# twesterhout/annealing-sign-problem

Hardware: AMD Instinct MI355X
Metric: SA spin-flips/sec, kagome_36-sized clusters (higher is better)
Workload: dtype f64

## Files before the change

annealing_sign_problem_amd/_lib.py:

```python
from __future__ import annotations

import atexit
import ctypes
import os
import sys
import weakref
from typing import Optional

import numpy as np

from . import build as _build

c_void_p = ctypes.c_void_p
c_u64 = ctypes.c_uint64
c_u32 = ctypes.c_uint32
c_i32 = ctypes.c_int32
c_int = ctypes.c_int
c_float = ctypes.c_float
c_double = ctypes.c_double


class AspError(RuntimeError):

    def __init__(self, code: int, message: str):
# ... 187 lines not shown
                                       ctypes.c_double, c_u64, c_void_p, ctypes.POINTER(c_u64),
                                       c_u64, c_void_p, c_void_p, c_void_p, ctypes.POINTER(c_u64)]),
    "asp_sparsify_last_ms": (c_float, []),
    "asp_sa_plan_create": (c_void_p, [c_u64, c_void_p, c_void_p, c_void_p, c_void_p]),
    "asp_sa_plan_destroy": (None, [c_void_p]),
    "asp_sa_plan_info": (c_int, [c_void_p, ctypes.POINTER(SaInfo)]),
    "asp_sa_layout_host": (c_int, [c_u64, c_void_p, c_void_p, c_void_p, c_void_p,
                                   ctypes.POINTER(SaInfo), c_void_p, c_void_p]),
    "asp_sa_layout_build_count": (c_u64, []),
    "asp_sa_plan_reweight": (c_int, [c_void_p, c_u64, c_void_p, c_void_p, c_void_p, c_void_p]),
    "asp_sa_plan_reweight_last_ms": (c_float, [c_void_p]),
    "asp_sa_plan_clone": (c_int, [c_void_p, ctypes.POINTER(c_void_p)]),
    "asp_sa_batch_slots_host": (c_int, [c_u32, c_void_p, c_void_p, ctypes.POINTER(c_u32), c_void_p, c_u64]),
    "asp_sa_shuffled_order_host": (c_int, [c_u64, c_void_p, c_void_p, c_void_p, c_void_p, c_u64, c_u32,
                                           c_void_p, c_void_p, ctypes.POINTER(c_u32)]),
    "asp_sa_set_launch": (c_int, [c_void_p, c_int, c_int]),
    "asp_sa_set_packed": (c_int, [c_void_p, c_int]),
    "asp_sa_set_wide": (c_int, [c_void_p, c_int]),
    "asp_sa_set_team": (c_int, [c_void_p, c_int]),
    "asp_sa_last_layout": (c_int, [c_void_p]),
    "asp_sa_set_lds_limit": (c_int, [c_void_p, c_u64]),
    "asp_sa_last_spin_layout": (c_int, [c_void_p]),
    "asp_sa_set_field_cache": (c_int, [c_void_p, c_int]),
    "asp_sa_set_post": (c_int, [c_void_p, c_int]),
    "asp_sa_anneal": (c_int, [c_void_p, c_u64, c_void_p, c_u32, c_u32, c_u32, c_void_p, c_void_p,
                              c_void_p]),
    "asp_sa_anneal_trace": (c_int, [c_void_p, c_u64, c_void_p, c_u32, c_u32, c_u32, c_void_p,
                                    c_void_p, c_void_p, c_void_p]),
    "asp_sa_anneal_shuffled": (c_int, [c_void_p, c_u64, c_void_p, c_u32, c_u32, c_u32, c_void_p, c_void_p,
                                       c_void_p]),
    "asp_sa_anneal_shuffled_trace": (c_int, [c_void_p, c_u64, c_void_p, c_u32, c_u32, c_u32, c_void_p,
                                             c_void_p, c_void_p, c_void_p]),
    "asp_sa_set_shuffled_launch": (c_int, [c_void_p, c_int, c_int]),
    "asp_sa_set_shuffled_teams": (c_int, [c_void_p, c_int]),
    "asp_sa_last_shuffled": (c_int, [c_void_p, ctypes.POINTER(c_u32), ctypes.POINTER(c_float)]),
    "asp_sa_team_watchdog_trips": (c_int, [c_void_p, ctypes.POINTER(c_u32), ctypes.POINTER(c_u64)]),
    "asp_sa_last_shuffled_blocks": (c_int, [c_void_p, ctypes.POINTER(c_u32), ctypes.POINTER(c_u32)]),
    "asp_sa_last_shuffled_fill": (c_int, [c_void_p, ctypes.POINTER(ctypes.c_double), ctypes.POINTER(ctypes.c_double)]),
    "asp_sa_chains_create": (c_int, [c_void_p, c_u64, c_u32, c_u32, c_void_p, c_u64, ctypes.POINTER(c_void_p)]),
    "asp_sa_chains_destroy": (None, [c_void_p]),
    "asp_sa_chains_advance": (c_int, [c_void_p, c_void_p, c_u32, c_u32, c_void_p]),
    "asp_sa_chains_result": (c_int, [c_void_p, c_void_p, c_void_p]),
    "asp_sa_chains_export": (c_int, [c_void_p, ctypes.POINTER(SaChainsSnapshot)]),
    "asp_sa_chains_import": (c_int, [c_void_p, ctypes.POINTER(SaChainsSnapshot)]),
    "asp_sa_chains_advance_batch": (c_int, [ctypes.POINTER(SaChainsItem), c_u32]),
    "asp_sa_chains_batch_last_ms": (c_float, []),
    "asp_sa_chains_gather": (c_int, [c_void_p, c_void_p]),
    "asp_sa_chains_resample": (c_int, [c_void_p, c_double, c_u32, c_void_p, c_void_p, c_void_p, c_void_p]),
# ... 170 lines not shown
```

annealing_sign_problem_amd/annealer.py:

```python
from __future__ import annotations

import ctypes
import os
from typing import Optional, Tuple

import numpy as np
import scipy.sparse

from . import _lib

__all__ = [
    "Hamiltonian",
    "PatternMismatch",
    "anneal",
    "anneal_batch",
    "anneal_traces",
    "anneal_until",
    "Chains",
    "resample_chains",
    "population_anneal",
    "population_anneal_batch",
    "parallel_tempering",
    "parallel_tempering_batch",
    "parallel_tempering_cluster",
# ... 218 lines not shown
def _resolve_seed(seed) -> int:
    if seed is None:
        return int.from_bytes(os.urandom(8), "little")
    return int(seed) & (2**64 - 1)


def anneal_raw(hamiltonian: Hamiltonian, seed: int, betas: np.ndarray, repetitions: int,
               replica_offset: int = 0, x0=None, shuffled: bool = False):
    lib = _lib.load()
    plan = hamiltonian.plan()
    words = (hamiltonian.size + 63) // 64
    betas = np.ascontiguousarray(betas, dtype=np.float64)
    xs = np.zeros((repetitions, max(words, 1)), dtype=np.uint64)
    es = np.zeros(repetitions, dtype=np.float64)
    if x0 is not None:
        x0 = np.ascontiguousarray(x0, dtype=np.uint64).reshape(-1)
        if x0.shape[0] != words:
            raise ValueError("'x0' must have {} words".format(words))
    entry = lib.asp_sa_anneal_shuffled if shuffled else lib.asp_sa_anneal
    _lib.check(entry(plan, ctypes.c_uint64(seed), _lib.ptr(betas),
                     ctypes.c_uint32(betas.shape[0]), ctypes.c_uint32(repetitions),
                     ctypes.c_uint32(replica_offset), _lib.ptr(x0), _lib.ptr(xs), _lib.ptr(es)))
    return xs[:, :words], es


def anneal_raw_into(hamiltonian: Hamiltonian, seed: int, betas: np.ndarray, repetitions: int,
                    replica_offset: int, x0, out_x_ptr: int, out_e_ptr: int,
                    shuffled: bool = False) -> None:
    lib = _lib.load()
    betas = np.ascontiguousarray(betas, dtype=np.float64)
    if x0 is not None:
        x0 = np.ascontiguousarray(x0, dtype=np.uint64).reshape(-1)
        if x0.shape[0] != (hamiltonian.size + 63) // 64:
            raise ValueError("'x0' must have {} words".format((hamiltonian.size + 63) // 64))
    entry = lib.asp_sa_anneal_shuffled if shuffled else lib.asp_sa_anneal
    _lib.check(entry(hamiltonian.plan(), ctypes.c_uint64(seed), _lib.ptr(betas),
                     ctypes.c_uint32(betas.shape[0]), ctypes.c_uint32(repetitions),
                     ctypes.c_uint32(replica_offset), _lib.ptr(x0),
                     ctypes.c_void_p(out_x_ptr), ctypes.c_void_p(out_e_ptr)))


def anneal(hamiltonian: Hamiltonian, x0=None, seed=None, number_sweeps: int = 5120,
           beta0: Optional[float] = None, beta1: Optional[float] = None, repetitions: int = 1,
           only_best: bool = True, distributed: bool = True, sweep_order: Optional[str] = None):
    if not isinstance(hamiltonian, Hamiltonian):
        raise TypeError("'hamiltonian' must be a Hamiltonian")
# ... 762 lines not shown
```

annealing_sign_problem_amd/csrc/sa_internal.hpp:

```cpp
#pragma once

#include <hip/hip_runtime.h>

#include <algorithm>
#include <atomic>
#include <cstdint>
#include <memory>
#include <mutex>
#include <utility>
#include <vector>

#include "asp_common.hpp"
#include "sa_plan.hpp"

namespace asp {

struct SaPattern {
  uint64_t nnz = 0;
  std::vector<int64_t> indptr;
  std::vector<int32_t> indices;
  std::mutex build;
  bool built = false;
  static constexpr uint32_t kNone = 0xFFFFFFFFu;
  std::vector<uint32_t> src_ij, src_ji;
// ... 30 lines not shown
  size_t spin_lds() const { return spin_lds_limit ? std::min(spin_lds_limit, max_lds) : max_lds; }
  asp::DeviceBuffer<uint32_t> color_block_start, block_width, ell_col, spin_of_pos, pos_of_spin;
  asp::DeviceBuffer<uint32_t> ell_col4;
  int last_layout = 0;
  int last_spin_layout = 0;
  asp::DeviceBuffer<uint64_t> ell_off;
  asp::DeviceBuffer<double> ell_val, field_pos;
  asp::DeviceBuffer<double> w_betas, w_partial, w_e;
  asp::DeviceBuffer<uint64_t> w_best, w_x0, w_x0_perm, w_x;
  asp::DeviceBuffer<long long> w_tracked;
  asp::DeviceBuffer<unsigned long long> w_accepted;
  asp::DeviceBuffer<double> w_field_cache;
  asp::DeviceBuffer<uint64_t> w_spins;
  asp::DeviceBuffer<long long> w_trace;
  asp::DeviceBuffer<uint64_t> w_cur_perm;
  asp::DeviceBuffer<long long> w_e_cur;
  void *team_area = nullptr;
  size_t team_area_bytes = 0;
  ~asp_sa_plan() {
    if (team_area) (void)hipFree(team_area);
  }
  int team_mode = -1;
  bool use_field_cache = true;
  bool use_post = true;
  uint32_t team_abort_host = 0;
  uint32_t team_watchdog_trips = 0;
  asp::DeviceBuffer<uint32_t> rq_ptr;
  asp::DeviceBuffer<uint32_t> rq_col;
  asp::DeviceBuffer<double> rq_val;
  asp::DeviceBuffer<double> field_dev;
  uint32_t rq_quads = 0, rq_max_quads = 0;
  int shuffled_m = 0, shuffled_waves = 0;
  int shuffled_teams = 0;
  int last_shuffled_levels = 0;
  uint32_t last_shuffled_log_s = 6, last_shuffled_wgs = 0;
  uint32_t last_shuffled_blocks = 0, last_shuffled_quads = 0;
  float last_order_ms = 0.0f;
  asp::DeviceBuffer<uint32_t> cluster_row_ptr, cluster_col;
  asp::DeviceBuffer<double> cluster_val, cluster_field;
  asp::DeviceBuffer<uint32_t> cluster_scratch;
  int greedy_tree = 0;
};


struct asp_sa_chains {
  asp_sa_plan *plan = nullptr;
// ... 99 lines not shown
```

annealing_sign_problem_amd/csrc/sa_reweight.hip:

```cpp
#include <hip/hip_runtime.h>

#include <algorithm>
#include <cmath>
#include <cstring>
#include <limits>
#include <vector>

#include "asp_common.hpp"
#include "sa_internal.hpp"

namespace {

using asp::SaPattern;

constexpr uint32_t kNone = SaPattern::kNone;
constexpr int kThreads = 256;

__global__ __launch_bounds__(kThreads) void k_rw_merge(const double *__restrict__ data,
                                                       const uint32_t *__restrict__ src_ij,
                                                       const uint32_t *__restrict__ src_ji, uint64_t entries,
                                                       double *__restrict__ staged, uint32_t *zeros) {
  const uint64_t stride = static_cast<uint64_t>(gridDim.x) * kThreads;
  for (uint64_t e = static_cast<uint64_t>(blockIdx.x) * kThreads + threadIdx.x; e < entries; e += stride) {
    const uint32_t a = src_ij[e], b = src_ji[e];
// ... 284 lines not shown
  ASP_HIP_TRY(hipEventElapsedTime(&p->rw_last_ms, p->ev[0], p->ev[3]));
  return ASP_OK;
}

float asp_sa_plan_reweight_last_ms(asp_sa_plan const *p) { return p ? p->rw_last_ms : 0.0f; }

int asp_sa_plan_clone(asp_sa_plan const *p, asp_sa_plan **out) {
  asp_clear_error();
  if (!p) return asp::set_error(ASP_ERR_INVALID, "null plan");
  if (!out) return asp::set_error(ASP_ERR_INVALID, "null output pointer");
  *out = nullptr;
  ASP_TRY(asp::bind_device());
  asp_sa_plan *c = new (std::nothrow) asp_sa_plan();
  if (!c) return asp::set_error(ASP_ERR_ALLOC, "out of host memory");
  c->host = p->host;
  c->pattern = p->pattern;
  c->force_m = p->force_m;
  c->force_threads = p->force_threads;
  c->force_packed = p->force_packed;
  c->spin_lds_limit = p->spin_lds_limit;
  c->allow_wide = p->allow_wide;
  c->team_mode = p->team_mode;
  c->use_field_cache = p->use_field_cache;
  c->use_post = p->use_post;
  c->shuffled_m = p->shuffled_m;
  c->shuffled_waves = p->shuffled_waves;
  c->shuffled_teams = p->shuffled_teams;
  c->greedy_tree = p->greedy_tree;
  const int rc = asp::sa_plan_device_setup(c);
  if (rc != ASP_OK) {
    asp_sa_plan_destroy(c);
    return rc;
  }
  *out = c;
  return ASP_OK;
}

}
```

annealing_sign_problem_amd/csrc/sa_sweep.hip:

```cpp
#include <algorithm>
#include <atomic>
#include <chrono>
#include <cmath>
#include <cstdlib>
#include <initializer_list>
#include <memory>
#include <mutex>
#include <numeric>
#include <type_traits>
#include <vector>

#include "asp_common.hpp"
#include "greedy.hpp"
#include "sa_device.hpp"
#include "sa_internal.hpp"
#include "sa_plan.hpp"

namespace {

using asp::DeviceBuffer;
using asp::kDummySpin;
using asp::upload_vector;
using namespace asp::dev;

// ... 311 lines not shown
  __device__ __forceinline__ double of(int, double beta) const { return beta; }
};
template <int M>
struct LadderBetas<M, true> {
  static constexpr bool kHeld = M <= 2;
  double own[kHeld ? M : 1];
  const double *mine;
  __device__ __forceinline__ LadderBetas(const ResumeLadder &res, uint32_t group)
      : mine(res.chain_betas + static_cast<uint64_t>(group) * M) {
    if constexpr (kHeld) {
#pragma unroll
      for (int m = 0; m < M; ++m) own[m] = mine[m];
    }
  }
  __device__ __forceinline__ double of(int m, double) const {
    if constexpr (kHeld) {
      return own[m];
    } else {
      return mine[m];
    }
  }
};

template <int M, bool DESCENT, int LAYOUT, typename Args, typename Stop = NoEarlyStop,
          typename Res = NoResume, bool ALIGNED = false>
__device__ __forceinline__ void sa_sweep_body(const Args &a, const uint32_t group,
                                              const Stop stop = Stop{}, const Res res = Res{}) {
  static_assert(DESCENT || !Stop::kEnabled, "only a descent can stop early");
  static_assert(!ALIGNED || (!DESCENT && M == 4), "an aligned group is one whole Philox call");
  static_assert(!DESCENT || !Res::kEnabled, "a descent is never resumed");
  constexpr bool GLOBAL = LAYOUT == kGlobal;
  constexpr bool PACKED = LAYOUT == kBits || GLOBAL;
  constexpr bool WIDE = LAYOUT == kWide;
  constexpr bool NIBBLES = LAYOUT == kNibbles;
  constexpr bool kLeanBook = M <= 4 && !(Res::kLadder && WIDE);
  static_assert(!PACKED || M == 1, "the bit-packed layouts hold one replica");
  static_assert(!NIBBLES || (M <= 4 && !DESCENT), "the nibble layout holds up to four replicas");
  static_assert(!WIDE || (M <= 4 && !DESCENT), "the wide layout holds up to four replicas");
  extern __shared__ __align__(16) uint8_t lds[];
  uint8_t *spins = GLOBAL ? reinterpret_cast<uint8_t *>(a.spin_words +
                                                       static_cast<uint64_t>(group) * a.num_blocks)
                          : lds;
  const uint32_t P = GLOBAL ? 0u : a.num_blocks * (PACKED ? 8u : (WIDE ? 256u : (NIBBLES ? 32u : 64u)));
  long long *delta = reinterpret_cast<long long *>(lds + P);
  long long *book = delta + 8;
  uint32_t *improved_flag = reinterpret_cast<uint32_t *>(book + 24);
  uint2 *meta = reinterpret_cast<uint2 *>(book + 26);
  uint32_t *cache_ctl = reinterpret_cast<uint32_t *>(meta + (PACKED ? 0u : a.num_blocks));
  uint8_t *dirty = reinterpret_cast<uint8_t *>(cache_ctl + 4);
  uint8_t *inert = dirty + ((a.num_blocks + 15u) & ~15u);
  const bool cache_available = !PACKED && a.field_cache != nullptr;

  if (reinterpret_cast<uintptr_t>((__attribute__((address_space(3))) uint8_t *)lds) != 0) {
    __builtin_trap();
  }
  const uint32_t tid = threadIdx.x;
  const uint32_t lane = tid & 63u;
  const uint32_t wave = tid >> 6;
  const uint32_t waves = blockDim.x >> 6;
  const uint32_t r0 = a.replica_first + group * M;
  const uint32_t key0 = static_cast<uint32_t>(a.seed);
  const uint32_t key1 = static_cast<uint32_t>(a.seed >> 32);

  for (uint32_t b0 = tid >> 6; b0 < a.num_blocks; b0 += blockDim.x >> 6) {
    const uint32_t p = b0 * 64u + (tid & 63u);
    const uint32_t spin = a.spin_of_pos[p];
    uint32_t byte = 0;
    if constexpr (Res::kEnabled) {
      if (spin != kDummySpin) {
#pragma unroll
        for (int m = 0; m < M; ++m) {
          const uint64_t word = res.cur_perm[(static_cast<uint64_t>(group) * M + m) * a.num_blocks + b0];
          byte |= static_cast<uint32_t>((word >> (tid & 63u)) & 1ull) << replica_bit<M, LAYOUT>(m);
        }
// ... 41 lines not shown
      meta[b] = make_uint2(static_cast<uint32_t>(a.ell_off[b]), a.block_width[b]);
    }
  }
  if constexpr (Res::kEnabled) {
    if (tid < 32) {
      const uint32_t which = tid >> 3, m = tid & 7u;
      long long v = 0;
      if (which >= 1u && m < static_cast<uint32_t>(M)) {
        const uint64_t chain = static_cast<uint64_t>(group) * M + m;
        v = which == 1u ? res.e_cur[chain]
                        : (which == 2u ? a.tracked[chain] : static_cast<long long>(a.accepted[chain]));
      }
      delta[tid] = v;
    }
  } else {
    if (tid < 32) delta[tid] = 0;
  }
  if (tid == 0) {
    *improved_flag = 0;
    cache_ctl[0] = 0;
    cache_ctl[1] = 0;
    cache_ctl[2] = 0;
    cache_ctl[3] = 0;
  }
  if constexpr (Res::kEnabled) {
    __syncthreads();
  } else {
    __syncthreads();
    snapshot<M, LAYOUT>(spins, a, group, (1u << M) - 1u);
    __syncthreads();
  }

  if (a.trace != nullptr && tid < M) {
    long long start = 0;
    if constexpr (Res::kEnabled) start = book[tid];
    a.trace[(static_cast<uint64_t>(group) * M + tid) * (a.num_sweeps + 1ull)] = start;
  }
  double mult[4] = {1.0, 1.0, 1.0, 1.0};
  const LadderBetas<M, Res::kLadder> ladder(res, group);
  [[maybe_unused]] uint32_t sweeps_done = a.num_sweeps;
  [[maybe_unused]] long long flips_before = 0;
  uint32_t ticket_base = 0;
  for (uint32_t t = 0; t < a.num_sweeps; ++t) {
    uint32_t t_draw = t;
    if constexpr (Res::kEnabled) t_draw += res.t0;
    double beta;
    if constexpr (DESCENT || Res::kLadder) {
      beta = 0.0;
    } else {
      beta = a.betas[t];
    }
    const bool cached = cache_available && __builtin_amdgcn_readfirstlane(cache_ctl[1]) != 0;
    if constexpr (!DESCENT && !Res::kLadder) {
      if (cached && t > 0 && beta < a.betas[t - 1]) {
        for (uint32_t b = tid; b < a.num_blocks; b += blockDim.x) inert[b] = 0;
        __syncthreads();
      }
    }
    unsigned long long q_acc[M];
    uint32_t n_acc[M];
    [[maybe_unused]] uint32_t visits = 0;
#pragma unroll
    for (int m = 0; m < M; ++m) {
      q_acc[m] = 0;
      n_acc[m] = 0;
    }

    for (uint32_t c = 0; c < a.num_colors; ++c) {
      const uint32_t b_begin = a.color_block_start[c];
      const uint32_t b_end = a.color_block_start[c + 1];
      uint32_t ticket = 0;
      for (uint32_t b = b_begin + wave; b < b_end;
           b = b_begin + waves + (__builtin_amdgcn_readfirstlane(ticket) - ticket_base)) {
        if (lane == 0) ticket = atomicInc(&cache_ctl[3], 0xFFFFFFFFu);
        const uint32_t p = b * 64u + lane;
        bool reuse = false;
        if (cached) {
          reuse = (__builtin_amdgcn_readfirstlane(static_cast<uint32_t>(dirty[b])) &
                   ((1u << M) - 1u)) == 0u;
          if (reuse && __builtin_amdgcn_readfirstlane(static_cast<uint32_t>(inert[b])) != 0u) {
            continue;
          }
        }
        if constexpr (kLeanBook) visits += 1;
        const uint2 info =
            PACKED ? make_uint2(static_cast<uint32_t>(a.ell_off[b]), a.block_width[b]) : meta[b];
        const uint32_t quads = __builtin_amdgcn_readfirstlane(info.y) >> 2;
        const uint64_t first_quad = __builtin_amdgcn_readfirstlane(info.x) >> 2;
        const uint4 *col = reinterpret_cast<const uint4 *>(a.ell_col) + first_quad * 64u;
        const double2 *val = reinterpret_cast<const double2 *>(a.ell_val) + first_quad * 128u;
        const BlockStream stream{col + lane, block_rsrc(col), block_rsrc(val), lane * 16u};
// ... 163 lines not shown
    {
      uint32_t any = 0;
#pragma unroll
      for (int m = 0; m < M; ++m) any |= n_acc[m];
      if (__ballot(any != 0) != 0ull) {
#pragma unroll
        for (int m0 = 0; m0 < M; m0 += 2) {
          unsigned long long v[2] = {0, 0};
#pragma unroll
          for (int j = 0; j < 2 && m0 + j < M; ++j) {
            v[j] = wave_sum_lane63_u64(
                kLeanBook ? q_acc[m0 + j] - visits * 0x4338000000000000ull : q_acc[m0 + j]);
          }
          const unsigned long long n2 = wave_sum_lane63_u64(
              n_acc[m0] | (m0 + 1 < M ? static_cast<unsigned long long>(n_acc[m0 + 1 < M ? m0 + 1 : m0]) << 32 : 0ull));
          if (lane == 63) {
#pragma unroll
            for (int j = 0; j < 2 && m0 + j < M; ++j) {
              const uint32_t n = static_cast<uint32_t>(n2 >> (32 * j));
              if (n != 0) {
                atomicAdd(reinterpret_cast<unsigned long long *>(&delta[m0 + j]), v[j]);
                atomicAdd(reinterpret_cast<unsigned long long *>(&book[16 + m0 + j]),
                          static_cast<unsigned long long>(n));
                if (cache_available) atomicAdd(&cache_ctl[0], n);
              }
            }
          }
        }
      }
    }
    __syncthreads();
    if (cache_available && tid == 0) {
      const uint32_t flips = cache_ctl[0];
      cache_ctl[0] = 0;
      const bool was = cache_ctl[1] != 0;
      const bool now = was ? flips < 2u * a.cache_enter_flips : flips < a.cache_enter_flips;
      cache_ctl[1] = now ? 1u : 0u;
      cache_ctl[2] = (now && !was) ? 1u : 0u;
    }
    if (tid < M) {
      const long long e = book[tid] + delta[tid];
      book[tid] = e;
      delta[tid] = 0;
      if (a.trace != nullptr) {
        a.trace[(static_cast<uint64_t>(group) * M + tid) * (a.num_sweeps + 1ull) + t + 1u] = e;
      }
      if (e < book[8 + tid]) {
        book[8 + tid] = e;
        atomicOr(improved_flag, 1u << tid);
      }
    }
    __syncthreads();
    if constexpr (DESCENT && Stop::kEnabled) {
      static_assert(M == 1, "one chain decides when the workgroup stops");
      const long long flips = book[16];
      if (flips == flips_before) {
        sweeps_done = t + 1u;
        break;
      }
      flips_before = flips;
    }
    const uint32_t improved = DESCENT ? ((1u << M) - 1u) : *improved_flag;
    if (improved) snapshot<M, LAYOUT>(spins, a, group, improved);
    if (cache_available && cache_ctl[2] != 0) {
      for (uint32_t b = tid; b < a.num_blocks; b += blockDim.x) dirty[b] = 0xFF;
    }
    __syncthreads();
    if (tid == 0) {
      *improved_flag = 0;
      if (cache_available) cache_ctl[2] = 0;
    }
  }

  if (tid < M) {
    a.tracked[static_cast<uint64_t>(group) * M + tid] = book[8 + tid];
    a.accepted[static_cast<uint64_t>(group) * M + tid] =
        static_cast<unsigned long long>(book[16 + tid]);
  }
  if constexpr (DESCENT && Stop::kEnabled) {
    if (tid == 0) *stop.sweeps_done = sweeps_done;
  }
  if constexpr (Res::kEnabled) {
    if (tid < M) res.e_cur[static_cast<uint64_t>(group) * M + tid] = book[tid];
    if constexpr (std::is_same_v<Args, SweepArgs>) {
      SweepArgs fin = a;
      fin.best_perm = res.cur_perm;
      snapshot<M, LAYOUT>(spins, fin, group, (1u << M) - 1u);
    } else {
      struct FinalWords {
        uint64_t *best_perm;
        uint32_t num_blocks;
      };
      const FinalWords fin{res.cur_perm, a.num_blocks};
      snapshot<M, LAYOUT>(spins, fin, group, (1u << M) - 1u);
    }
  }
}

template <int M, bool DESCENT, int LAYOUT, bool ALIGNED = false>
__global__ __launch_bounds__(kMaxThreads) void k_sa_sweep(SweepArgs a) {
  sa_sweep_body<M, DESCENT, LAYOUT, SweepArgs, NoEarlyStop, NoResume, ALIGNED>(a, blockIdx.x);
}

template <int M, int LAYOUT, typename Res>
__global__ __launch_bounds__(kMaxThreads) void k_sa_sweep_resume(SweepArgs a, Res r) {
  sa_sweep_body<M, false, LAYOUT, SweepArgs, NoEarlyStop, Res>(a, blockIdx.x, NoEarlyStop{}, r);
}

struct BatchSlot {
  uint32_t problem;
  uint32_t group;
};
template <typename Problem>
struct BatchArgs {
  const Problem *problems;
  const BatchSlot *slots;
  uint32_t slots_per_xcd;
};

struct DescentProblem {
  SweepArgs s;
  const uint64_t *x0;
  uint64_t *x0_perm;
  uint32_t *sweeps_done;
// ... 751 lines not shown
  };
  (take(Forms{}), ...);
  return kernel;
}
template <typename Family>
typename Family::Kernel colour_kernel_of(int m, int layout) {
  return colour_kernel_in<Family>(ColourForms{}, m, layout);
}
ClosedFamily<false, false>::Kernel closed_kernel_of(int m, bool descent, int layout, uint32_t replica_first) {
  if (descent) return colour_kernel_of<ClosedFamily<true, false>>(m, layout);
  if (aligned_replicas(m, replica_first)) return colour_kernel_of<ClosedFamily<false, true>>(m, layout);
  return colour_kernel_of<ClosedFamily<false, false>>(m, layout);
}

size_t sweep_lds_bytes(const asp::SaHostLayout &L, int layout) {
  if (layout == kGlobal) return 34 * sizeof(long long) + 32;
  if (layout == kBits) return static_cast<size_t>(L.num_blocks) * 8 + 34 * sizeof(long long) + 32;
  const size_t per_block = layout == kWide ? 256 : (layout == kNibbles ? 32 : 64);
  return static_cast<size_t>(L.num_blocks) * per_block + 34 * sizeof(long long) +
         static_cast<size_t>(L.num_blocks) * sizeof(uint2) + 16 +
         2 * (((static_cast<size_t>(L.num_blocks) + 15) / 16) * 16);
}

size_t team_lds_bytes(const asp::SaHostLayout &L) {
  return static_cast<size_t>(L.num_blocks) * 8 + 64 +
         2 * (((static_cast<size_t>(L.num_blocks) + 15) / 16) * 16);
}

uint32_t widest_color(const asp::SaHostLayout &L) {
  uint32_t widest = 1;
  for (uint32_t c = 0; c < L.num_colors; ++c) {
    widest = std::max(widest, L.color_block_start[c + 1] - L.color_block_start[c]);
  }
  return widest;
}

void choose_launch(const asp_sa_plan *p, uint32_t repetitions, int *m_out, int *threads_out) {
  const uint32_t widest = widest_color(p->host);
  int m = 1;
  bool two_per_cu = false;
  if (p->force_m) {
    m = p->force_m;
  } else {
    for (int cand : {8, 4, 2}) {
      if ((repetitions + cand - 1) / cand >= static_cast<uint32_t>(p->num_cus)) {
        m = cand;
// ... 242 lines not shown
  info->beta1_auto = L.beta1_auto;
  return ASP_OK;
}

int asp_sa_set_launch(asp_sa_plan *p, int replicas_per_group, int threads) {
  if (!p) return asp::set_error(ASP_ERR_INVALID, "null plan");
  if (replicas_per_group != 0 && !colour_form_exists(replicas_per_group, kBytes)) {
    return asp::set_error(ASP_ERR_INVALID, "replicas_per_group must be 0, 1, 2, 4 or 8");
  }
  if (threads != 0 && (threads < 64 || threads > 1024 || threads % 64 != 0)) {
    return asp::set_error(ASP_ERR_INVALID, "threads must be 0 or a multiple of 64 in [64, 1024]");
  }
  p->force_m = replicas_per_group;
  p->force_threads = threads;
  return ASP_OK;
}

int asp_sa_set_field_cache(asp_sa_plan *p, int enable) {
  if (!p) return asp::set_error(ASP_ERR_INVALID, "null plan");
  p->use_field_cache = enable != 0;
  return ASP_OK;
}

int asp_sa_set_post(asp_sa_plan *p, int enable) {
  if (!p) return asp::set_error(ASP_ERR_INVALID, "null plan");
  p->use_post = enable != 0;
  return ASP_OK;
}

int asp_sa_team_watchdog_trips(asp_sa_plan const *p, uint32_t *of_plan, uint64_t *of_process) {
  if (of_plan) *of_plan = p ? p->team_watchdog_trips : 0u;
  if (of_process) *of_process = g_team_watchdog_trips.load(std::memory_order_relaxed);
  return ASP_OK;
}

int asp_sa_set_team(asp_sa_plan *p, int team) {
  if (!p) return asp::set_error(ASP_ERR_INVALID, "null plan");
  if (team != -1 && team != 0 && team != 2 && team != 4 && team != 8) {
    return asp::set_error(ASP_ERR_INVALID, "team must be -1 (auto), 0 (off), 2, 4 or 8");
  }
  p->team_mode = team;
  return ASP_OK;
}

int asp_sa_set_wide(asp_sa_plan *p, int allow) {
  if (!p) return asp::set_error(ASP_ERR_INVALID, "null plan");
// ... 13 lines not shown

int asp_sa_set_packed(asp_sa_plan *p, int packed) {
  if (!p) return asp::set_error(ASP_ERR_INVALID, "null plan");
  p->force_packed = packed < 0 ? 0 : (packed > 2 ? 2 : packed);
  return ASP_OK;
}

}

namespace {

int greedy_relax(asp_sa_plan *p, uint32_t max_sweeps, std::vector<uint64_t> &x, uint64_t *out_x,
                 double *out_e, uint32_t *out_sweeps, bool exact_sweeps);

struct ColourRun {
  asp_sa_plan *p;
  uint32_t repetitions, num_sweeps;
  int64_t *trace;
  int m = 1, threads = 64, layout = kBytes;
  size_t lds = 0;
  uint32_t groups = 0;
  uint64_t padded = 0;
  SweepArgs args{};

  int shape(const ColourLaunch &form, size_t lds_bytes) {
    m = form.m, threads = form.threads, layout = form.layout, lds = lds_bytes;
    if (lds > p->max_lds) {
      return asp::set_error(ASP_ERR_TOO_LARGE, "%zu B of LDS needed, %zu B available", lds, p->max_lds);
    }
    groups = (repetitions + m - 1) / m;
    padded = static_cast<uint64_t>(groups) * m;
    return ASP_OK;
  }
  int ensure_work(uint64_t num_betas) {
    if (layout == kGlobal) ASP_TRY(p->w_spins.ensure(static_cast<uint64_t>(groups) * p->host.num_blocks));
    ASP_TRY(p->w_betas.ensure(num_betas));
    ASP_TRY(p->w_best.ensure(padded * p->host.num_blocks));
    ASP_TRY(p->w_tracked.ensure(padded));
    return p->w_accepted.ensure(padded);
  }
  int fill(const double *betas, const uint64_t *x0_perm, uint64_t seed, uint32_t replica_first) {
    args = sweep_args(p, layout, betas, x0_perm, p->w_best.ptr, p->w_tracked.ptr, p->w_accepted.ptr, seed,
                      num_sweeps, replica_first);
    if (trace) {
      ASP_TRY(p->w_trace.ensure(padded * (static_cast<uint64_t>(num_sweeps) + 1)));
      args.trace = p->w_trace.ptr;
    }
    if (p->use_field_cache && !bit_packed(layout)) attach_field_cache(p, padded, &args);
    return ASP_OK;
  }
  template <typename Kernel, typename... Extra>
  int launch(Kernel kernel, Extra... extra) {
    if (!kernel) return asp::set_error(ASP_ERR_INVALID, "no sweep kernel for %d chains per group", m);
    ASP_TRY(asp::allow_dynamic_lds(reinterpret_cast<const void *>(kernel), lds));
    ASP_HIP_TRY(hipEventRecord(p->ev[1], p->stream));
    hipLaunchKernelGGL(kernel, dim3(groups), dim3(threads), lds, p->stream, args, extra...);
    ASP_HIP_TRY(hipGetLastError());
    ASP_HIP_TRY(hipEventRecord(p->ev[2], p->stream));
    return ASP_OK;
  }
  int collect() {
    if (trace) {
      ASP_HIP_TRY(hipMemcpyAsync(trace, p->w_trace.ptr,
                                 static_cast<uint64_t>(repetitions) * (num_sweeps + 1ull) * sizeof(int64_t),
                                 hipMemcpyDeviceToHost, p->stream));
    }
    ASP_HIP_TRY(hipStreamSynchronize(p->stream));
    return ASP_OK;
  }
  int record(int launch_layout) {
    p->last_m = m;
// ... 77 lines not shown
  p->last_sweep_ms = p->last_total_ms = 0.0f;
  if (K == 0) {
    for (uint32_t r = 0; r < repetitions; ++r) out_e[r] = 0.0;
    return ASP_OK;
  }
  ColourLaunch form = choose_colour_launch(p, repetitions, descent, out_trace != nullptr);
  uint32_t team = 0;
  {
    const uint32_t widest = widest_color(L);
    const bool possible = !out_trace && form.layout != kGlobal && form.layout != kNibbles && p->force_packed == 0 &&
                          L.num_colors >= 2 && p->force_m == 0 && team_lds_bytes(L) <= p->max_lds &&
                          static_cast<uint64_t>(repetitions) * 2 <= static_cast<uint64_t>(p->num_cus);
    if (possible && p->team_mode >= 2) {
      team = static_cast<uint32_t>(p->team_mode);
    } else if (possible && p->team_mode < 0 && widest >= 64) {
      const uint32_t spare = static_cast<uint32_t>(p->num_cus) / repetitions;
      team = spare >= 8 ? 8u : (spare >= 4 ? 4u : 2u);
      while (team > 2 && widest < 16u * team) team >>= 1;
    }
    if (team * repetitions > static_cast<uint32_t>(p->num_cus)) team = 0;
  }
  if (team >= 2) form.m = 1, form.layout = kBits;
  ColourRun run{p, repetitions, num_sweeps, out_trace};
  ASP_TRY(run.shape(form, team >= 2 ? team_lds_bytes(L) : sweep_lds_bytes(L, form.layout)));
  hipStream_t s = p->stream;
  asp::StreamFence fence(s);
  ASP_TRY(run.ensure_work(num_sweeps));
  ASP_TRY(p->w_partial.ensure(static_cast<uint64_t>(repetitions) * L.num_blocks));
  ASP_TRY(p->w_e.ensure(repetitions));
  ASP_TRY(p->w_x.ensure(static_cast<uint64_t>(repetitions) * words));
  ASP_TRY(p->w_betas.upload(betas, num_sweeps, s));
  ASP_HIP_TRY(hipMemsetAsync(p->w_accepted.ptr, 0, run.padded * sizeof(unsigned long long), s));
  if (x0) {
    ASP_TRY(p->w_x0.ensure(words));
    ASP_TRY(p->w_x0_perm.ensure(L.num_blocks));
    ASP_TRY(p->w_x0.upload(x0, words, s));
    ASP_TRY(asp::sa_permute_bits(p, p->w_x0.ptr, 1u, p->w_x0_perm.ptr));
  }
  ASP_TRY(run.fill(p->w_betas.ptr, x0 ? p->w_x0_perm.ptr : nullptr, seed, replica_offset));

  p->team_abort_host = 0;
  std::unique_lock<std::mutex> team_turn(g_team_launches, std::defer_lock);
  if (team >= 2) {
    team_turn.lock();
    bool refused = false;
    ASP_TRY(launch_team(run, team, descent, &refused));
    if (refused) {
      ASP_HIP_TRY(hipStreamSynchronize(s));
      team_turn.unlock();
      p->team_mode = 0;
      return run_chains(p, seed, betas, num_sweeps, repetitions, replica_offset, x0, descent, out_x,
                        out_e, out_trace);
    }
  } else {
    ASP_HIP_TRY(hipEventRecord(p->ev[0], s));
    ASP_TRY(run.launch(closed_kernel_of(run.m, descent, run.layout, replica_offset)));
  }
  ASP_TRY(energies_of_perm(p, p->w_best.ptr, repetitions, p->w_partial.ptr, p->w_e.ptr, p->w_x.ptr));
  ASP_HIP_TRY(hipEventRecord(p->ev[3], s));
  ASP_HIP_TRY(hipMemcpyAsync(out_x, p->w_x.ptr, static_cast<uint64_t>(repetitions) * words * sizeof(uint64_t),
                             hipMemcpyDefault, s));
  ASP_HIP_TRY(hipMemcpyAsync(out_e, p->w_e.ptr, repetitions * sizeof(double), hipMemcpyDefault, s));
  p->last_tracked.assign(repetitions, 0);
  p->last_accepted.assign(repetitions, 0);
  ASP_HIP_TRY(hipMemcpyAsync(p->last_tracked.data(), p->w_tracked.ptr, repetitions * sizeof(int64_t),
                             hipMemcpyDeviceToHost, s));
  ASP_HIP_TRY(hipMemcpyAsync(p->last_accepted.data(), p->w_accepted.ptr,
                             repetitions * sizeof(uint64_t), hipMemcpyDeviceToHost, s));
  ASP_TRY(run.collect());
  if (p->team_abort_host != 0) {
    if (team_turn.owns_lock()) team_turn.unlock();
    p->team_mode = 0;
    p->team_watchdog_trips += 1;
    g_team_watchdog_trips.fetch_add(1, std::memory_order_relaxed);
    return run_chains(p, seed, betas, num_sweeps, repetitions, replica_offset, x0, descent, out_x,
                      out_e, out_trace);
  }
  return run.record(team >= 2 ? 4 : run.layout);
}
// ... 1107 lines not shown
```

include/asp.h:

```cpp
#ifndef ASP_H
#define ASP_H

#include <stdint.h>

#ifdef __cplusplus
extern "C" {
#endif


typedef enum asp_status {
  ASP_OK = 0,
  ASP_ERR_NO_DEVICE = -1,
  ASP_ERR_HIP = -2,
  ASP_ERR_INVALID = -3,
  ASP_ERR_TOO_LARGE = -4,
  ASP_ERR_ALLOC = -5
} asp_status;

const char *asp_last_error(void);
int asp_last_error_code(void);
void asp_clear_error(void);

int asp_device_count(void);
int asp_device_touched(void);
// ... 145 lines not shown

int asp_sa_batch_slots_host(uint32_t count, double const *work, uint32_t const *groups,
                            uint32_t *slots_per_xcd, uint32_t *slots, uint64_t capacity);

int asp_sa_shuffled_order_host(uint64_t num_spins, int64_t const *indptr, int32_t const *indices,
                               double const *data, double const *field, uint64_t seed,
                               uint32_t sweep, uint32_t *order, uint32_t *level_of_position,
                               uint32_t *num_levels);

int asp_sa_set_launch(asp_sa_plan *p, int replicas_per_group, int threads);

int asp_sa_set_packed(asp_sa_plan *p, int packed);

int asp_sa_set_wide(asp_sa_plan *p, int allow);
int asp_sa_last_layout(asp_sa_plan const *p);
int asp_sa_set_lds_limit(asp_sa_plan *p, uint64_t bytes);
int asp_sa_last_spin_layout(asp_sa_plan const *p);

int asp_sa_set_team(asp_sa_plan *p, int team);
int asp_sa_team_watchdog_trips(asp_sa_plan const *p, uint32_t *of_plan, uint64_t *of_process);

int asp_sa_set_field_cache(asp_sa_plan *p, int enable);

int asp_sa_set_post(asp_sa_plan *p, int enable);

int asp_sa_anneal(asp_sa_plan *p, uint64_t seed, double const *betas,
                  uint32_t num_sweeps, uint32_t repetitions, uint32_t replica_offset,
                  uint64_t const *x0, uint64_t *out_x, double *out_e);
int asp_sa_anneal_trace(asp_sa_plan *p, uint64_t seed, double const *betas, uint32_t num_sweeps,
                        uint32_t repetitions, uint32_t replica_offset, uint64_t const *x0,
                        uint64_t *out_x, double *out_e, int64_t *out_trace);

int asp_sa_anneal_shuffled(asp_sa_plan *p, uint64_t seed, double const *betas, uint32_t num_sweeps,
                           uint32_t repetitions, uint32_t replica_offset, uint64_t const *x0,
                           uint64_t *out_x, double *out_e);
int asp_sa_anneal_shuffled_trace(asp_sa_plan *p, uint64_t seed, double const *betas,
                                 uint32_t num_sweeps, uint32_t repetitions,
                                 uint32_t replica_offset, uint64_t const *x0, uint64_t *out_x,
                                 double *out_e, int64_t *out_trace);
int asp_sa_set_shuffled_launch(asp_sa_plan *p, int chains_per_group, int wavefronts);
int asp_sa_set_shuffled_teams(asp_sa_plan *p, int teams);
int asp_sa_last_shuffled(asp_sa_plan const *p, uint32_t *levels, float *order_ms);
int asp_sa_last_shuffled_blocks(asp_sa_plan const *p, uint32_t *spins_per_block, uint32_t *workgroups);
int asp_sa_last_shuffled_fill(asp_sa_plan const *p, double *lane_fill, double *row_fill);

typedef struct asp_sa_chains asp_sa_chains;
// ... 159 lines not shown
```

Measured before the change: 311.2 billion.

## Add tail-mode sweeps that revisit only spins near flipped neighbours

Adds a tail kernel variant for four-chain byte/word layouts. Once the per-sweep flip count drops below a threshold derived from spin count and degree, sweeps visit only spins marked in an LDS todo bitmap, compacted through per-wave rings. A spin stays marked while its acceptance is still plausible, and flips mark their neighbours. This replaces the field cache when active, and it costs extra LDS, atomics and ring-compaction overhead while changing which spins get visited.

```diff
diff --git a/annealing_sign_problem_amd/_lib.py b/annealing_sign_problem_amd/_lib.py
--- a/annealing_sign_problem_amd/_lib.py
+++ b/annealing_sign_problem_amd/_lib.py
@@ -233,8 +233,10 @@
     "asp_sa_set_lds_limit": (c_int, [c_void_p, c_u64]),
     "asp_sa_last_spin_layout": (c_int, [c_void_p]),
     "asp_sa_set_field_cache": (c_int, [c_void_p, c_int]),
+    "asp_sa_set_tail": (c_int, [c_void_p, c_int]),
+    "asp_sa_last_tail": (c_int, [c_void_p, ctypes.POINTER(c_u32), ctypes.POINTER(c_u32), ctypes.POINTER(c_u32)]),
     "asp_sa_set_post": (c_int, [c_void_p, c_int]),
-    "asp_sa_anneal": (c_int, [c_void_p, c_u64, c_void_p, c_u32, c_u32, c_u32, c_void_p, c_void_p,
+    "asp_sa_anneal":(c_int, [c_void_p, c_u64, c_void_p, c_u32, c_u32, c_u32, c_void_p, c_void_p,
                               c_void_p]),
     "asp_sa_anneal_trace": (c_int, [c_void_p, c_u64, c_void_p, c_u32, c_u32, c_u32, c_void_p,
                                     c_void_p, c_void_p, c_void_p]),
diff --git a/annealing_sign_problem_amd/annealer.py b/annealing_sign_problem_amd/annealer.py
--- a/annealing_sign_problem_amd/annealer.py
+++ b/annealing_sign_problem_amd/annealer.py
@@ -264,6 +264,16 @@
                      ctypes.c_uint32(betas.shape[0]), ctypes.c_uint32(repetitions),
                      ctypes.c_uint32(replica_offset), _lib.ptr(x0), _lib.ptr(xs), _lib.ptr(es)))
     return xs[:, :words], es
+
+
+def set_tail(hamiltonian: Hamiltonian, n: int = -1) -> None:
+    _lib.check(_lib.load().asp_sa_set_tail(hamiltonian.plan(), int(n)))
+
+
+def last_tail(hamiltonian: Hamiltonian):
+    out = [ctypes.c_uint32(0) for _ in range(3)]
+    _lib.check(_lib.load().asp_sa_last_tail(hamiltonian.plan(), *[ctypes.byref(v) for v in out]))
+    return tuple(int(v.value) for v in out)
 
 
 def anneal_raw_into(hamiltonian: Hamiltonian, seed: int, betas: np.ndarray, repetitions: int,
diff --git a/annealing_sign_problem_amd/csrc/sa_internal.hpp b/annealing_sign_problem_amd/csrc/sa_internal.hpp
--- a/annealing_sign_problem_amd/csrc/sa_internal.hpp
+++ b/annealing_sign_problem_amd/csrc/sa_internal.hpp
@@ -76,6 +76,9 @@
   }
   int team_mode = -1;
   bool use_field_cache = true;
+  int tail_mode = -1;
+  asp::DeviceBuffer<uint32_t> w_tail;
+  std::vector<uint32_t> last_tail;
   bool use_post = true;
   uint32_t team_abort_host = 0;
   uint32_t team_watchdog_trips = 0;
diff --git a/annealing_sign_problem_amd/csrc/sa_reweight.hip b/annealing_sign_problem_amd/csrc/sa_reweight.hip
--- a/annealing_sign_problem_amd/csrc/sa_reweight.hip
+++ b/annealing_sign_problem_amd/csrc/sa_reweight.hip
@@ -330,6 +330,7 @@
   c->allow_wide = p->allow_wide;
   c->team_mode = p->team_mode;
   c->use_field_cache = p->use_field_cache;
+  c->tail_mode = p->tail_mode;
   c->use_post = p->use_post;
   c->shuffled_m = p->shuffled_m;
   c->shuffled_waves = p->shuffled_waves;
diff --git a/annealing_sign_problem_amd/csrc/sa_sweep.hip b/annealing_sign_problem_amd/csrc/sa_sweep.hip
--- a/annealing_sign_problem_amd/csrc/sa_sweep.hip
+++ b/annealing_sign_problem_amd/csrc/sa_sweep.hip
@@ -357,10 +357,19 @@
   }
 };
 
+struct TailArgs {
+  uint32_t enter_flips;
+  uint32_t *report;
+};
+constexpr uint32_t kTailRing = 128;
+
 template <int M, bool DESCENT, int LAYOUT, typename Args, typename Stop = NoEarlyStop,
-          typename Res = NoResume, bool ALIGNED = false>
+          typename Res = NoResume, bool ALIGNED = false, bool TAIL = false>
 __device__ __forceinline__ void sa_sweep_body(const Args &a, const uint32_t group,
-                                              const Stop stop = Stop{}, const Res res = Res{}) {
+                                              const Stop stop = Stop{}, const Res res = Res{},
+                                              const TailArgs tail = TailArgs{}) {
+  static_assert(!TAIL || (M == 4 && !DESCENT && !Res::kEnabled && (LAYOUT == kBytes || LAYOUT == kWide)),
+                "tail sweeps: the closed call of four chains in bytes or words");
   static_assert(DESCENT || !Stop::kEnabled, "only a descent can stop early");
   static_assert(!ALIGNED || (!DESCENT && M == 4), "an aligned group is one whole Philox call");
   static_assert(!DESCENT || !Res::kEnabled, "a descent is never resumed");
@@ -384,7 +393,9 @@
   uint32_t *cache_ctl = reinterpret_cast<uint32_t *>(meta + (PACKED ? 0u : a.num_blocks));
   uint8_t *dirty = reinterpret_cast<uint8_t *>(cache_ctl + 4);
   uint8_t *inert = dirty + ((a.num_blocks + 15u) & ~15u);
-  const bool cache_available = !PACKED && a.field_cache != nullptr;
+  const bool cache_available = !TAIL && !PACKED && a.field_cache != nullptr;
+  [[maybe_unused]] uint64_t *todo = reinterpret_cast<uint64_t *>(cache_ctl + 8);
+  [[maybe_unused]] uint32_t *todo32 = reinterpret_cast<uint32_t *>(todo);
 
   if (reinterpret_cast<uintptr_t>((__attribute__((address_space(3))) uint8_t *)lds) != 0) {
     __builtin_trap();
@@ -472,6 +483,7 @@
     cache_ctl[1] = 0;
     cache_ctl[2] = 0;
     cache_ctl[3] = 0;
+    if constexpr (TAIL) cache_ctl[4] = cache_ctl[5] = 0;
   }
   if constexpr (Res::kEnabled) {
     __syncthreads();
@@ -516,7 +528,177 @@
       n_acc[m] = 0;
     }
 
-    for (uint32_t c = 0; c < a.num_colors; ++c) {
+    uint32_t first_hot_colour = 0;
+    if constexpr (TAIL) {
+      if (__builtin_amdgcn_readfirstlane(cache_ctl[1]) != 0) {
+        const uint32_t wave_u = __builtin_amdgcn_readfirstlane(wave);
+        uint32_t *ring = reinterpret_cast<uint32_t *>(todo + a.num_blocks) + wave_u * kTailRing;
+        const BufferRsrc col_rsrc = block_rsrc(a.ell_col), val_rsrc = block_rsrc(a.ell_val);
+        for (uint32_t c = 0; c < a.num_colors; ++c) {
+          const uint32_t b_begin = a.color_block_start[c];
+          const uint32_t nb = a.color_block_start[c + 1] - b_begin;
+          uint32_t fill = 0, drained = 0;
+          uint32_t base = 0, next_base = wave_u;
+          uint64_t w = 0, nonempty = 0;
+          for (;;) {
+            while (fill - drained < 64u) {
+              if (nonempty == 0ull) {
+                if (next_base >= nb) break;
+                base = next_base;
+                next_base += waves * 64u;
+                const uint32_t i = base + lane * waves;
+                w = 0;
+                if (i < nb) {
+                  w = todo[b_begin + i];
+                  if (w != 0ull) todo[b_begin + i] = 0ull;
+                }
+                nonempty = __ballot(w != 0ull);
+                continue;
+              }
+              const uint32_t src = static_cast<uint32_t>(__builtin_ctzll(nonempty));
+              nonempty &= nonempty - 1ull;
+              const uint32_t w_lo = __builtin_amdgcn_readlane(static_cast<uint32_t>(w), src);
+              const uint32_t w_hi = __builtin_amdgcn_readlane(static_cast<uint32_t>(w >> 32), src);
+              const uint32_t rank = __builtin_amdgcn_mbcnt_hi(w_hi, __builtin_amdgcn_mbcnt_lo(w_lo, 0u));
+              const uint32_t mine = lane < 32u ? w_lo >> lane : w_hi >> (lane - 32u);
+              if (mine & 1u) ring[(fill + rank) & (kTailRing - 1u)] = (b_begin + base + src * waves) * 64u + lane;
+              fill += static_cast<uint32_t>(__builtin_popcount(w_lo) + __builtin_popcount(w_hi));
+            }
+            const uint32_t count = min(64u, fill - drained);
+            if (count == 0u) break;
+            __builtin_amdgcn_fence(__ATOMIC_ACQ_REL, "wavefront");
+            const bool live = lane < count;
+            uint32_t p = 0, row_quads = 0, col_at = 0, val_at = 0;
+            if (live) {
+              p = ring[(drained + lane) & (kTailRing - 1u)];
+              const uint2 info = meta[p >> 6];
+              row_quads = info.y >> 2;
+              col_at = (info.x >> 2) * 1024u + (p & 63u) * 16u;
+              val_at = (info.x >> 2) * 2048u + (p & 63u) * 16u;
+            }
+            drained += count;
+            visits += 1;
+            uint32_t spin = kDummySpin;
+            double h = 0.0;
+            if constexpr (!WIDE) {
+              if (live) {
+                spin = a.spin_of_pos[p];
+                h = a.field_pos[p];
+              }
+            }
+            auto load_row_quad = [&](Quad &q, uint32_t quad) {
+              const bool mine = quad < row_quads;
+              const uint32_t c_at = mine ? col_at + quad * 1024u : 0u;
+              const uint32_t v_at = mine ? val_at + quad * 2048u : 0u;
+              q.c = __builtin_bit_cast(uint4, __builtin_amdgcn_raw_buffer_load_b128(col_rsrc, c_at, 0, 0));
+              q.v01 = __builtin_bit_cast(double2, __builtin_amdgcn_raw_buffer_load_b128(val_rsrc, v_at, 0, 0));
+              q.v23 = __builtin_bit_cast(double2,
+                                         __builtin_amdgcn_raw_buffer_load_b128(val_rsrc, v_at + (mine ? 1024u : 16u), 0, 0));
+            };
+            double acc[M];
+#pragma unroll
+            for (int m = 0; m < M; ++m) acc[m] = 0.0;
+            Quad qa, qb;
+            load_row_quad(qa, 0u);
+            for (uint32_t q = 0; __ballot(q < row_quads) != 0ull; q += 2u) {
+              load_row_quad(qb, q + 1u);
+              __builtin_amdgcn_sched_barrier(0);
+              if (q < row_quads) accumulate<M, LAYOUT>(qa, spins, acc, mult);
+              __builtin_amdgcn_sched_barrier(0);
+              load_row_quad(qa, q + 2u);
+              __builtin_amdgcn_sched_barrier(0);
+              if (q + 1u < row_quads) accumulate<M, LAYOUT>(qb, spins, acc, mult);
+              __builtin_amdgcn_sched_barrier(0);
+            }
+            uint32_t own = 0;
+            if (live) {
+              if constexpr (WIDE) {
+                spin = a.spin_of_pos[p];
+                h = a.field_pos[p];
+              }
+              if constexpr (WIDE) {
+                own = reinterpret_cast<const uint32_t *>(spins)[p];
+              } else {
+                own = spins[p];
+              }
+            }
+            const bool valid = spin != kDummySpin;
+            bool open = false, need = false;
+            double de[M];
+#pragma unroll
+            for (int m = 0; m < M; ++m) {
+              const double g = __dadd_rn(acc[m], h);
+              const bool negative = (own >> (WIDE ? 8 * m + 7 : replica_bit<M, LAYOUT>(m))) & 1u;
+              de[m] = __dmul_rn(negative ? 2.0 : -2.0, g);
+              const bool maybe = valid && !(__dmul_rn(beta, de[m]) >= 23.0);
+              open = open || maybe;
+              need = need || (maybe && !(de[m] <= 0.0));
+            }
+            uint32_t took[M];
+            if (__ballot(need) != 0ull) {
+              Philox4 rnd{};
+              uint32_t have = 0xFFFFFFFFu;
+#pragma unroll
+              for (int m = 0; m < M; ++m) {
+                uint32_t word;
+                if constexpr (ALIGNED) {
+                  if (m == 0) rnd = philox4x32_10(spin, t_draw, r0 >> 2, 0u, key0, key1);
+                  word = rnd.w[m];
+                } else {
+                  const uint32_t r = r0 + m;
+                  if (m == 0 || (r >> 2) != have) {
+                    have = r >> 2;
+                    rnd = philox4x32_10(spin, t_draw, have, 0u, key0, key1);
+                  }
+                  word = pick_word(rnd, r & 3u);
+                }
+                const bool accept =
+                    valid && (de[m] <= 0.0 || metropolis_accept_word(word, __dmul_rn(beta, de[m])));
+                took[m] = accept ? 0xFFFFFFFFu : 0u;
+              }
+            } else {
+#pragma unroll
+              for (int m = 0; m < M; ++m) took[m] = (valid && de[m] <= 0.0) ? 0xFFFFFFFFu : 0u;
+            }
+            uint32_t flip = 0;
+            double round_bias = 0x1.8p52;
+            asm volatile("" : "+v"(round_bias));
+            const uint32_t scale_hi = static_cast<uint32_t>(__double2hiint(a.scale));
+#pragma unroll
+            for (int m = 0; m < M; ++m) {
+              flip |= took[m] & (1u << m);
+              const double scale_m = __hiloint2double(static_cast<int>(scale_hi & took[m]), 0);
+              q_acc[m] += static_cast<unsigned long long>(
+                  __double_as_longlong(__builtin_fma(de[m], scale_m, round_bias)));
+              n_acc[m] -= took[m];
+            }
+            if (open) atomicOr(&todo32[p >> 5], 1u << (p & 31u));
+            if (flip) {
+              if constexpr (WIDE) {
+                reinterpret_cast<uint32_t *>(spins)[p] = own ^ spread_mask(flip);
+              } else {
+                spins[p] = static_cast<uint8_t>(own ^ encode_replicas<M, LAYOUT>(flip));
+              }
+              const uint4 *cols4 = reinterpret_cast<const uint4 *>(
+                  reinterpret_cast<const uint8_t *>(a.ell_col) + col_at);
+              for (uint32_t q = 0; q < row_quads; ++q) {
+                const uint4 c4 = cols4[q * 64u];
+                const uint32_t cols[4] = {c4.x, c4.y, c4.z, c4.w};
+#pragma unroll
+                for (int j = 0; j < 4; ++j) {
+                  const uint32_t at = WIDE ? cols[j] >> 2 : cols[j];
+                  if (at != p) atomicOr(&todo32[at >> 5], 1u << (at & 31u));
+                }
+              }
+            }
+          }
+          __syncthreads();
+        }
+        first_hot_colour = a.num_colors;
+      }
+    }
+
+    for (uint32_t c = first_hot_colour; c < a.num_colors; ++c) {
       const uint32_t b_begin = a.color_block_start[c];
       const uint32_t b_end = a.color_block_start[c + 1];
       uint32_t ticket = 0;
@@ -726,7 +908,7 @@
                 atomicAdd(reinterpret_cast<unsigned long long *>(&delta[m0 + j]), v[j]);
                 atomicAdd(reinterpret_cast<unsigned long long *>(&book[16 + m0 + j]),
                           static_cast<unsigned long long>(n));
-                if (cache_available) atomicAdd(&cache_ctl[0], n);
+                if (TAIL || cache_available) atomicAdd(&cache_ctl[0], n);
               }
             }
           }
@@ -742,6 +924,19 @@
       cache_ctl[1] = now ? 1u : 0u;
       cache_ctl[2] = (now && !was) ? 1u : 0u;
     }
+    if constexpr (TAIL) {
+      if (tid == 0) {
+        const uint32_t flips = cache_ctl[0];
+        cache_ctl[0] = 0;
+        const bool was = cache_ctl[1] != 0;
+        bool now = was ? flips <= 2ull * tail.enter_flips : flips < tail.enter_flips;
+        if (t + 1u < a.num_sweeps && a.betas[t + 1u] < beta) now = false;
+        cache_ctl[1] = now ? 1u : 0u;
+        cache_ctl[2] = (now && !was) ? 1u : 0u;
+        if (was) cache_ctl[4] += 1u;
+        if (now && !was) cache_ctl[5] += 1u;
+      }
+    }
     if (tid < M) {
       const long long e = book[tid] + delta[tid];
       book[tid] = e;
@@ -769,10 +964,21 @@
     if (cache_available && cache_ctl[2] != 0) {
       for (uint32_t b = tid; b < a.num_blocks; b += blockDim.x) dirty[b] = 0xFF;
     }
+    if constexpr (TAIL) {
+      if (cache_ctl[2] != 0) {
+        for (uint32_t b = tid; b < a.num_blocks; b += blockDim.x) todo[b] = ~0ull;
+      }
+    }
     __syncthreads();
     if (tid == 0) {
       *improved_flag = 0;
-      if (cache_available) cache_ctl[2] = 0;
+      if (TAIL || cache_available) cache_ctl[2] = 0;
+    }
+  }
+  if constexpr (TAIL) {
+    if (tid == 0) {
+      tail.report[2ull * group] = cache_ctl[4];
+      tail.report[2ull * group + 1u] = cache_ctl[5];
     }
   }
 
@@ -804,6 +1010,12 @@
 template <int M, bool DESCENT, int LAYOUT, bool ALIGNED = false>
 __global__ __launch_bounds__(kMaxThreads) void k_sa_sweep(SweepArgs a) {
   sa_sweep_body<M, DESCENT, LAYOUT, SweepArgs, NoEarlyStop, NoResume, ALIGNED>(a, blockIdx.x);
+}
+
+template <int LAYOUT, bool ALIGNED>
+__global__ __launch_bounds__(kMaxThreads) void k_sa_sweep_tail(SweepArgs a, TailArgs tail) {
+  sa_sweep_body<4, false, LAYOUT, SweepArgs, NoEarlyStop, NoResume, ALIGNED, true>(a, blockIdx.x, NoEarlyStop{},
+                                                                                    NoResume{}, tail);
 }
 
 template <int M, int LAYOUT, typename Res>
@@ -1601,6 +1813,32 @@
          2 * (((static_cast<size_t>(L.num_blocks) + 15) / 16) * 16);
 }
 
+size_t tail_lds_bytes(const asp::SaHostLayout &L, int layout, int threads) {
+  const size_t per_block = layout == kWide ? 256 : 64;
+  return static_cast<size_t>(L.num_blocks) * per_block + 34 * sizeof(long long) +
+         static_cast<size_t>(L.num_blocks) * sizeof(uint2) + 32 + static_cast<size_t>(L.num_blocks) * sizeof(uint64_t) +
+         static_cast<size_t>(threads / 64) * kTailRing * sizeof(uint32_t);
+}
+
+constexpr double kTailEnterShare = 0.05;
+uint32_t tail_enter_flips_of(const asp::SaHostLayout &L) {
+  const double degree = std::max(1.0, static_cast<double>(L.a_col.size()) / static_cast<double>(L.num_spins));
+  return static_cast<uint32_t>(std::max(1.0, kTailEnterShare * static_cast<double>(L.num_spins) / degree));
+}
+
+using TailKernel = void (*)(SweepArgs, TailArgs);
+TailKernel tail_kernel_of(const asp_sa_plan *p, int m, int threads, int layout, bool descent, uint32_t replica_first) {
+  const asp::SaHostLayout &L = p->host;
+  if (p->tail_mode == 0 || !p->use_field_cache || descent || m != 4 || (layout != kBytes && layout != kWide)) {
+    return nullptr;
+  }
+  if (tail_lds_bytes(L, layout, threads) > p->max_lds) return nullptr;
+  if (L.ell_val.size() * sizeof(double) >= (1ull << 32)) return nullptr;
+  const bool aligned = replica_first % 4u == 0;
+  if (layout == kWide) return aligned ? k_sa_sweep_tail<kWide, true> : k_sa_sweep_tail<kWide, false>;
+  return aligned ? k_sa_sweep_tail<kBytes, true> : k_sa_sweep_tail<kBytes, false>;
+}
+
 size_t team_lds_bytes(const asp::SaHostLayout &L) {
   return static_cast<size_t>(L.num_blocks) * 8 + 64 +
          2 * (((static_cast<size_t>(L.num_blocks) + 15) / 16) * 16);
@@ -1889,6 +2127,27 @@
   return ASP_OK;
 }
 
+int asp_sa_set_tail(asp_sa_plan *p, int n) {
+  if (!p) return asp::set_error(ASP_ERR_INVALID, "null plan");
+  if (n < -1) return asp::set_error(ASP_ERR_INVALID, "n must be -1 (auto), 0 (off) or a number of flips");
+  p->tail_mode = n;
+  return ASP_OK;
+}
+
+int asp_sa_last_tail(asp_sa_plan const *p, uint32_t *sweeps_min, uint32_t *sweeps_max, uint32_t *entries_max) {
+  if (!p) return asp::set_error(ASP_ERR_INVALID, "null plan");
+  uint32_t lo = p->last_tail.empty() ? 0u : 0xFFFFFFFFu, hi = 0, entries = 0;
+  for (size_t g = 0; g + 1 < p->last_tail.size(); g += 2) {
+    lo = std::min(lo, p->last_tail[g]);
+    hi = std::max(hi, p->last_tail[g]);
+    entries = std::max(entries, p->last_tail[g + 1]);
+  }
+  if (sweeps_min) *sweeps_min = lo;
+  if (sweeps_max) *sweeps_max = hi;
+  if (entries_max) *entries_max = entries;
+  return ASP_OK;
+}
+
 int asp_sa_set_post(asp_sa_plan *p, int enable) {
   if (!p) return asp::set_error(ASP_ERR_INVALID, "null plan");
   p->use_post = enable != 0;
@@ -1948,6 +2207,7 @@
   uint32_t groups = 0;
   uint64_t padded = 0;
   SweepArgs args{};
+  bool tail = false;
 
   int shape(const ColourLaunch &form, size_t lds_bytes) {
     m = form.m, threads = form.threads, layout = form.layout, lds = lds_bytes;
@@ -1972,7 +2232,7 @@
       ASP_TRY(p->w_trace.ensure(padded * (static_cast<uint64_t>(num_sweeps) + 1)));
       args.trace = p->w_trace.ptr;
     }
-    if (p->use_field_cache && !bit_packed(layout)) attach_field_cache(p, padded, &args);
+    if (p->use_field_cache && !bit_packed(layout) && !tail) attach_field_cache(p, padded, &args);
     return ASP_OK;
   }
   template <typename Kernel, typename... Extra>
@@ -2096,7 +2356,12 @@
   }
   if (team >= 2) form.m = 1, form.layout = kBits;
   ColourRun run{p, repetitions, num_sweeps, out_trace};
-  ASP_TRY(run.shape(form, team >= 2 ? team_lds_bytes(L) : sweep_lds_bytes(L, form.layout)));
+  const TailKernel tail_kernel =
+      team >= 2 ? nullptr : tail_kernel_of(p, form.m, form.threads, form.layout, descent, replica_offset);
+  run.tail = tail_kernel != nullptr;
+  ASP_TRY(run.shape(form, team >= 2 ? team_lds_bytes(L)
+                                    : (run.tail ? tail_lds_bytes(L, form.layout, form.threads)
+                                                : sweep_lds_bytes(L, form.layout))));
   hipStream_t s = p->stream;
   asp::StreamFence fence(s);
   ASP_TRY(run.ensure_work(num_sweeps));
@@ -2126,9 +2391,19 @@
       return run_chains(p, seed, betas, num_sweeps, repetitions, replica_offset, x0, descent, out_x,
                         out_e, out_trace);
     }
+  } else if (run.tail) {
+    ASP_TRY(p->w_tail.ensure(2ull * run.groups));
+    ASP_HIP_TRY(hipEventRecord(p->ev[0], s));
+    const uint32_t enter = p->tail_mode > 0 ? static_cast<uint32_t>(p->tail_mode) : tail_enter_flips_of(L);
+    ASP_TRY(run.launch(tail_kernel, TailArgs{enter, p->w_tail.ptr}));
   } else {
     ASP_HIP_TRY(hipEventRecord(p->ev[0], s));
     ASP_TRY(run.launch(closed_kernel_of(run.m, descent, run.layout, replica_offset)));
+  }
+  p->last_tail.assign(run.tail ? 2ull * run.groups : 0, 0u);
+  if (run.tail) {
+    ASP_HIP_TRY(hipMemcpyAsync(p->last_tail.data(), p->w_tail.ptr, p->last_tail.size() * sizeof(uint32_t),
+                               hipMemcpyDeviceToHost, s));
   }
   ASP_TRY(energies_of_perm(p, p->w_best.ptr, repetitions, p->w_partial.ptr, p->w_e.ptr, p->w_x.ptr));
   ASP_HIP_TRY(hipEventRecord(p->ev[3], s));
diff --git a/include/asp.h b/include/asp.h
--- a/include/asp.h
+++ b/include/asp.h
@@ -191,6 +191,9 @@
 
 int asp_sa_set_field_cache(asp_sa_plan *p, int enable);
 
+int asp_sa_set_tail(asp_sa_plan *p, int n);
+int asp_sa_last_tail(asp_sa_plan const *p, uint32_t *sweeps_min, uint32_t *sweeps_max, uint32_t *entries_max);
+
 int asp_sa_set_post(asp_sa_plan *p, int enable);
 
 int asp_sa_anneal(asp_sa_plan *p, uint64_t seed, double const *betas,
```

Measured after the change: 331.5 billion, median of 6. 6.5% higher.
